# josebeo2016/SCL-Deepfake-audio-detection

Measured on AMD Instinct MI355X. Metric: train-step utterances/sec (64000-sample clips), higher is better.
Workload: dtype bf16

## Files before the change

### scl-deepfake-audio-detection_amd/csrc/gemm.hip

```cpp
#include "gemm_common.h"

using namespace sclg;

namespace {

constexpr int BM = 128, BN = 128;

struct StageK {
    __amdgpu_buffer_rsrc_t rsrc;
    unsigned rowoff[4];
    unsigned lds_off[4];
    int kcur, kend;

    __device__ __forceinline__ void init(const OpK& o, const char* base, int row0, int rowlimit, int kbegin, int kend_, int tid) {
        rsrc = make_rsrc(base);
        const int c = tid & 7;
#pragma unroll
        for (int i = 0; i < 4; ++i) {
            const int row = (tid >> 3) + 32 * i;
            const int r = row0 + row;
            rowoff[i] = r < rowlimit ? row_off(o, (unsigned)r) : OOB;
            lds_off[i] = (unsigned)(row * 128 + ((c ^ ((row >> 1) & 7)) << 4));
        }
        kcur = kbegin + 8 * c; kend = kend_;
// ... 644 lines not shown

bool fill_operand(const SclOperand& o, const char* name, long long rows, long long contig, OpK* k, int esz) {
    const int vec = 16 / esz;
    if (!o.ptr || ((uintptr_t)o.ptr & 15)) { scl_set_error("gemm: %s ptr null or not 16B aligned", name); return false; }
    if (o.rpb < 1 || o.cin < vec) { scl_set_error("gemm: %s rpb/cin invalid", name); return false; }
    if ((o.ld % vec) || (o.rbstride % vec) || (o.cout % vec) || (o.bs1 % vec) || (o.bs2 % vec) || (o.cin != 0x7fffffff && (o.cin % vec))) {
        scl_set_error("gemm: %s strides must be multiples of %d elements", name, vec); return false;
    }
    const long long rq = (rows - 1) / o.rpb, rr = o.rpb == 0x7fffffff ? rows - 1 : (long long)o.rpb - 1;
    const long long cq = o.cin == 0x7fffffff ? 0 : (contig - 1) / o.cin;
    const long long cr = o.cin == 0x7fffffff ? contig - 1 : (long long)o.cin - 1;
    const long long maxoff = rq * o.rbstride + (rr < rows - 1 ? rr : rows - 1) * (long long)o.ld + cq * o.cout + cr + vec;
    if (maxoff < 0 || maxoff * esz >= (1ll << 32) - 32 || rows >= (1ll << 31)) {
        scl_set_error("gemm: %s extent exceeds 32-bit byte offsets (%lld elements)", name, maxoff); return false;
    }
    k->ptr = o.ptr; k->bs1 = o.bs1 * esz; k->bs2 = o.bs2 * esz;
    k->rb_bytes = (unsigned)(o.rbstride * esz); k->ld_bytes = (unsigned)o.ld * (unsigned)esz; k->cout_bytes = (unsigned)(o.cout * esz);
    k->rpb = (unsigned)o.rpb; make_magic((unsigned)o.rpb, &k->rpb_magic, &k->rpb_shift);
    k->cin = (unsigned)o.cin; make_magic((unsigned)o.cin, &k->cin_magic, &k->cin_mshift);
    k->esz_shift = esz == 4 ? 2u : 1u;
    return true;
}
}

namespace {

bool gemm_pick_w8(const GemmK& k, bool at, bool bt, const SclGemmDesc& d, long long zdim, W8Plan* plan) {
    const int w8_env = 1;
    if (d.flags & (SCL_GEMM_NO_W8 | SCL_GEMM_FORCE_P8 | SCL_GEMM_FORCE_BIG | SCL_GEMM_NO_DMA)) return false;
    const bool a_whole = at ? (d.M % 8 == 0) : (d.K % 8 == 0);
    const bool b_whole = bt ? (d.N % 8 == 0) : (d.K % 8 == 0);
    static const int ncu_env = [] { const char* e = getenv("SCL_GEMM_CUS"); const int v = e ? atoi(e) : 256; return v >= 32 && v <= 256 ? v : 256; }();
    if (!a_whole || !b_whole || !scl_gemm_w8_plan(k, at, bt, d, zdim, ncu_env, plan)) return false;
    const long long need = at ? 128 : 160;
    return (d.flags & SCL_GEMM_FORCE_W8) || (w8_env && d.N >= 192 && plan->tiles * zdim >= need);
}

#ifdef SCL_EXPERIMENTS
bool gemm_pick_x2(const GemmK& k, bool at, bool bt, const SclGemmDesc& d, long long zdim, W8Plan* plan) {
    static const int x2_env = [] { const char* e = getenv("SCL_GEMM_X2"); return e ? atoi(e) : 0; }();
    if (d.flags & (SCL_GEMM_NO_X2 | SCL_GEMM_FORCE_W8 | SCL_GEMM_FORCE_P8 | SCL_GEMM_FORCE_BIG | SCL_GEMM_NO_DMA)) return false;
    if (!(d.flags & SCL_GEMM_FORCE_X2) && x2_env == 0) return false;
    const bool a_whole = at ? (d.M % 8 == 0) : (d.K % 8 == 0);
    const bool b_whole = bt ? (d.N % 8 == 0) : (d.K % 8 == 0);
    static const int ncu_env = [] { const char* e = getenv("SCL_GEMM_CUS"); const int v = e ? atoi(e) : 256; return v >= 32 && v <= 256 ? v : 256; }();
    if (!a_whole || !b_whole || !scl_gemm_x2_plan(k, at, bt, d, zdim, ncu_env, plan)) return false;
    if ((d.flags & SCL_GEMM_FORCE_X2) || x2_env == 2) return true;
    return !at && d.N >= 128 && plan->tiles * zdim >= 248;
}

#else
bool gemm_pick_x2(const GemmK&, bool, bool, const SclGemmDesc&, long long, W8Plan*) { return false; }
#endif
}

extern "C" int scl_gemm_uses_wide_tiles(const SclGemmDesc* dp) {
    if (!dp || dp->M <= 0 || dp->N <= 0 || dp->K <= 0 || dp->nb1 < 1 || dp->nb2 < 1 || dp->splitk < 1) return 0;
    GemmK k; W8Plan plan;
    const bool at = dp->flags & SCL_GEMM_A_T, bt = dp->flags & SCL_GEMM_B_T;
    const long long zdim = (long long)dp->nb1 * dp->nb2 * dp->splitk;
    if (gemm_pick_x2(k, at, bt, *dp, zdim, &plan)) return 3;
    return gemm_pick_w8(k, at, bt, *dp, zdim, &plan) ? (plan.variant == 2 ? 4 : 1 + plan.variant) : 0;
}

static int gemm_colsum_rows(const SclGemmDesc& d) {
    if (d.M <= 0 || d.N <= 0 || d.K <= 0 || d.nb1 != 1 || d.nb2 != 1 || d.splitk != 1 || (d.N & 7) || (d.ldc & 7) || (d.flags & SCL_GEMM_AB_F32)) return 0;
    GemmK k; W8Plan plan;
    const bool at = d.flags & SCL_GEMM_A_T, bt = d.flags & SCL_GEMM_B_T;
    const bool a_whole = at ? (d.M % 8 == 0) : (d.K % 8 == 0), b_whole = bt ? (d.N % 8 == 0) : (d.K % 8 == 0);
    SclGemmDesc dq = d;
    if (!dq.colsum_part) dq.colsum_part = reinterpret_cast<float*>(16);
    if (!a_whole || !b_whole || (d.flags & SCL_GEMM_NO_DMA) || gemm_pick_x2(k, at, bt, dq, 1, &plan) || !gemm_pick_w8(k, at, bt, dq, 1, &plan)) return 0;
    return plan.tiles_m * 4;
}
extern "C" int scl_gemm_colsum_rows(const SclGemmDesc* dp) { return dp ? gemm_colsum_rows(*dp) : 0; }

static int gemm_fill_k(const SclGemmDesc& d, GemmK& k) {
    SCL_REQUIRE(d.M > 0 && d.N > 0 && d.K > 0, "gemm: M,N,K must be positive (%d,%d,%d)", d.M, d.N, d.K);
    SCL_REQUIRE(d.nb1 >= 1 && d.nb2 >= 1 && d.splitk >= 1, "gemm: nb1/nb2/splitk must be >= 1");
    const bool at = d.flags & SCL_GEMM_A_T, bt = d.flags & SCL_GEMM_B_T;
    const bool f32ab = d.flags & SCL_GEMM_AB_F32;
    if (!f32ab) {
        if (!fill_operand(d.A, "A", at ? d.K : d.M, at ? d.M : d.K, &k.A, 2)) return SCL_EINVAL;
        if (!fill_operand(d.B, "B", bt ? d.K : d.N, bt ? d.N : d.K, &k.B, 2)) return SCL_EINVAL;
    }
    SCL_REQUIRE(d.C && d.c_rpb >= 1, "gemm: C null or c_rpb < 1");
    const int rmode = (d.flags >> SCL_GEMM_RMODE_SHIFT) & 0xF;
    SCL_REQUIRE(rmode == 0 || d.R, "gemm: RMODE set but R is null");
    SCL_REQUIRE(!(d.flags & SCL_GEMM_HAS_C2) || d.C2, "gemm: HAS_C2 set but C2 is null");
    SCL_REQUIRE(!(d.flags & SCL_GEMM_HAS_BIAS) || d.bias, "gemm: HAS_BIAS set but bias is null");
    SCL_REQUIRE(d.splitk == 1 || ((d.flags & SCL_GEMM_C_F32) && rmode == 0 && !(d.flags & (SCL_GEMM_HAS_BIAS | SCL_GEMM_HAS_C2))
                                  && ((d.flags >> SCL_GEMM_ACT_SHIFT) & 0xF) == 0),
                "gemm: split-K needs a plain f32 slab output");
    const long long zdim = (long long)d.nb1 * d.nb2 * d.splitk;
    SCL_REQUIRE(zdim <= 65535, "gemm: batch*splitk too large (%lld)", zdim);
// ... 99 lines not shown
        return scl_check_launch("scl_gemm_bf16(f32 operands)");
    }
    {
        SclProfScope prof(SCL_KID_GEMM, s, 2.0 * d.M * d.N * (double)d.K * d.nb1 * d.nb2, true);
        const bool a_whole = at ? (d.M % 8 == 0) : (d.K % 8 == 0);
        const bool b_whole = bt ? (d.N % 8 == 0) : (d.K % 8 == 0);
        const bool dma = a_whole && b_whole && !(d.flags & SCL_GEMM_NO_DMA);
#ifdef SCL_EXPERIMENTS
        const long long big_tiles = (long long)((d.M + BIG_BM - 1) / BIG_BM) * ((d.N + BN - 1) / BN) * zdim;
        const bool big = dma && (d.flags & SCL_GEMM_FORCE_BIG) && !(d.flags & SCL_GEMM_NO_BIG) && d.M >= 256 && d.K >= 192 && big_tiles >= 1;
        const long long p8_tiles = (long long)((d.M + P8_BM - 1) / P8_BM) * ((d.N + P8_BN - 1) / P8_BN) * zdim;
        const bool p8 = dma && (d.flags & SCL_GEMM_FORCE_P8) && !(d.flags & SCL_GEMM_NO_P8);
#else
        const bool big = false, p8 = false;
#endif
        W8Plan plan;
#ifdef SCL_EXPERIMENTS
        const bool x2 = dma && gemm_pick_x2(k, at, bt, d, zdim, &plan);
#else
        const bool x2 = false;
#endif
        const bool w8 = !x2 && dma && gemm_pick_w8(k, at, bt, d, zdim, &plan);
        if (((unsigned)d.flags & SCL_GEMM_C_SPLIT3) && !w8) {
            scl_set_error("gemm: C_SPLIT3 is served by the wide-tile kernel only, and this launch (M %d, N %d, K %d) does not qualify for it", d.M, d.N, d.K);
            return SCL_EUNSUPPORTED;
        }
#ifdef SCL_EXPERIMENTS
        const char* deep_env = getenv("SCL_GEMM_DEEP");
        const bool deep = !x2 && !w8 && dma && deep_env && atoi(deep_env) != 0 && (long long)tiles * zdim <= 256 && (d.K + BK - 1) / BK / d.splitk >= 4;
#else
        const bool deep = false;
#endif
        const bool w8p = w8 && scl_gemm_w8_persist_blocks(k, at, bt, plan, zdim) > 0;
        prof.note(d.M, d.N, d.K, d.flags, (int)zdim, x2 ? 3 : (w8p ? 8 : (w8 ? (plan.variant == 2 ? 6 : 1 + plan.variant) : (deep ? 7 : 0))));
        if (x2) {
#ifdef SCL_EXPERIMENTS
            scl_gemm_x2_launch(k, at, bt, plan, zdim, s);
#endif
        } else if (w8) {
            scl_gemm_w8_launch(k, at, bt, plan, zdim, s);
#ifdef SCL_EXPERIMENTS
        } else if (p8) {
            static bool p8_attr_set = false;
            if (!p8_attr_set) {
                hipFuncSetAttribute((const void*)scl_gemm_p8_kernel<false, false>, hipFuncAttributeMaxDynamicSharedMemorySize, P8_LDS);
                hipFuncSetAttribute((const void*)scl_gemm_p8_kernel<false, true>, hipFuncAttributeMaxDynamicSharedMemorySize, P8_LDS);
                hipFuncSetAttribute((const void*)scl_gemm_p8_kernel<true, false>, hipFuncAttributeMaxDynamicSharedMemorySize, P8_LDS);
                hipFuncSetAttribute((const void*)scl_gemm_p8_kernel<true, true>, hipFuncAttributeMaxDynamicSharedMemorySize, P8_LDS);
                p8_attr_set = true;
            }
            dim3 pgrid((unsigned)(p8_tiles / zdim), 1, (unsigned)zdim), pblock(512);
            if (!at && !bt) SCL_LAUNCH((scl_gemm_p8_kernel<false, false>), pgrid, pblock, P8_LDS, s, k);
            else if (!at && bt) SCL_LAUNCH((scl_gemm_p8_kernel<false, true>), pgrid, pblock, P8_LDS, s, k);
            else if (at && !bt) SCL_LAUNCH((scl_gemm_p8_kernel<true, false>), pgrid, pblock, P8_LDS, s, k);
            else SCL_LAUNCH((scl_gemm_p8_kernel<true, true>), pgrid, pblock, P8_LDS, s, k);
        } else if (big) {
            static bool attr_set = false;
            if (!attr_set) {
                hipFuncSetAttribute((const void*)scl_gemm_big_kernel<false, false>, hipFuncAttributeMaxDynamicSharedMemorySize, BIG_LDS);
                hipFuncSetAttribute((const void*)scl_gemm_big_kernel<false, true>, hipFuncAttributeMaxDynamicSharedMemorySize, BIG_LDS);
                hipFuncSetAttribute((const void*)scl_gemm_big_kernel<true, false>, hipFuncAttributeMaxDynamicSharedMemorySize, BIG_LDS);
                hipFuncSetAttribute((const void*)scl_gemm_big_kernel<true, true>, hipFuncAttributeMaxDynamicSharedMemorySize, BIG_LDS);
                attr_set = true;
            }
            dim3 bgrid(((d.M + BIG_BM - 1) / BIG_BM) * ((d.N + BN - 1) / BN), 1, (unsigned)zdim), bblock(512);
            if (!at && !bt) SCL_LAUNCH((scl_gemm_big_kernel<false, false>), bgrid, bblock, BIG_LDS, s, k);
            else if (!at && bt) SCL_LAUNCH((scl_gemm_big_kernel<false, true>), bgrid, bblock, BIG_LDS, s, k);
// ... 138 lines not shown
```

### scl-deepfake-audio-detection_amd/csrc/gemm_w8.hip

```cpp
#include "gemm_common.h"
#include "gemm_w8_epi.h"

using namespace sclg;

__device__ unsigned long long scl_gemm_stamps[4096 * 8];

namespace {

__device__ __forceinline__ void w8_stamp(const GemmK& d, int slot, int lane, int wave) {
    if ((d.flags & SCL_GEMM_STAMPS) && wave == 0 && lane == 0 && blockIdx.x < 4096 && blockIdx.z == 0) {
        scl_gemm_stamps[blockIdx.x * 8 + 2 * slot] = __builtin_amdgcn_s_memrealtime();
        scl_gemm_stamps[blockIdx.x * 8 + 2 * slot + 1] = __builtin_amdgcn_s_memtime();
    }
}

constexpr int W8_BN = 256;
constexpr int W8_OPB = 2 * TILE_BYTES;
constexpr int W8_NA = 3, W8_NB = 2;
constexpr int W8_LDS = (W8_NA + W8_NB) * W8_OPB;

struct W8K {
    __amdgpu_buffer_rsrc_t rsrc;
    unsigned voff[4];
    __device__ __forceinline__ void init(const OpK& o, const char* base, int row0, int rowlimit, int lane, int wave) {
        rsrc = make_rsrc(base);
#pragma unroll
        for (int i = 0; i < 4; ++i) {
            const int row = 8 * (wave * 4 + i) + (lane >> 3);
            const int r = row0 + row;
            const int kc = (lane & 7) ^ ((row >> 1) & 7);
            voff[i] = r < rowlimit ? row_off(o, (unsigned)r) + (unsigned)(kc << 4) : OOB;
        }
    }
    template <int I0>
    __device__ __forceinline__ void issue2(char* img, int wave, unsigned soff, bool live) const {
#pragma unroll
        for (int i = I0; i < I0 + 2; ++i) {
            const unsigned off = live ? voff[i] : OOB;
            __builtin_amdgcn_raw_ptr_buffer_load_lds(rsrc, (lds_void*)(img + (wave * 4 + i) * 1024), 16, off, soff, 0, 0);
        }
    }
    __device__ __forceinline__ void issue1(char* img, int wave, unsigned soff, bool live, int i) const {
        const unsigned off = live ? voff[i] : OOB;
        __builtin_amdgcn_raw_ptr_buffer_load_lds(rsrc, (lds_void*)(img + (wave * 4 + i) * 1024), 16, off, soff, 0, 0);
    }
    __device__ __forceinline__ static unsigned kstep(const OpK& o) { return o.cin == 64 ? o.cout_bytes : 128u; }
    __device__ __forceinline__ void rows(const OpK&, int, int, int) {}
    __device__ __forceinline__ void set_batched(bool) {}
    __device__ __forceinline__ unsigned step(const OpK& o) const { return kstep(o); }
};
struct W8T {
    __amdgpu_buffer_rsrc_t rsrc;
    unsigned voff[4];
    int col0_, collimit_;
    bool batched;
    __device__ __forceinline__ void set_batched(bool b) { batched = b; }
    __device__ __forceinline__ void init(const OpK& o, const char* base, int col0, int collimit, int lane, int wave) {
        rsrc = make_rsrc(base);
        col0_ = col0; collimit_ = collimit;
        const int s16 = lane & 15;
#pragma unroll
        for (int i = 0; i < 4; ++i) {
            const int p = wave * 4 + i;
            const int kr = 4 * (p & 15) + (lane >> 4);
            const int sw = (kr & 3) | (((kr >> 3) & 1) << 2);
            const int col = col0 + (p >> 4) * 128 + 8 * ((((s16 >> 1) ^ sw) << 1) | (s16 & 1));
            voff[i] = col < collimit ? (unsigned)kr * o.ld_bytes + col_off(o, (unsigned)col) : OOB;
        }
    }
    __device__ __forceinline__ void rows(const OpK& o, int krow, int lane, int wave) {
        if (!batched) return;
        const int s16 = lane & 15;
#pragma unroll
        for (int i = 0; i < 4; ++i) {
            const int p = wave * 4 + i;
            const int kr = 4 * (p & 15) + (lane >> 4);
            const int sw = (kr & 3) | (((kr >> 3) & 1) << 2);
            const int col = col0_ + (p >> 4) * 128 + 8 * ((((s16 >> 1) ^ sw) << 1) | (s16 & 1));
            voff[i] = col < collimit_ ? row_off(o, (unsigned)(krow + kr)) + col_off(o, (unsigned)col) : OOB;
        }
    }
    template <int I0>
    __device__ __forceinline__ void issue2(char* img, int wave, unsigned soff, bool live) const {
#pragma unroll
        for (int i = I0; i < I0 + 2; ++i) {
            const unsigned off = live ? voff[i] : OOB;
            __builtin_amdgcn_raw_ptr_buffer_load_lds(rsrc, (lds_void*)(img + (wave * 4 + i) * 1024), 16, off, soff, 0, 0);
        }
    }
    __device__ __forceinline__ void issue1(char* img, int wave, unsigned soff, bool live, int i) const {
        const unsigned off = live ? voff[i] : OOB;
        __builtin_amdgcn_raw_ptr_buffer_load_lds(rsrc, (lds_void*)(img + (wave * 4 + i) * 1024), 16, off, soff, 0, 0);
    }
    __device__ __forceinline__ static unsigned kstep(const OpK& o) { return 64u * o.ld_bytes; }
    __device__ __forceinline__ unsigned step(const OpK& o) const { return batched ? 0u : kstep(o); }
};
template <bool T> struct W8Sel { typedef W8K type; };
template <> struct W8Sel<true> { typedef W8T type; };

template <bool T>
__device__ __forceinline__ bf16x8 w8_frag(const char* img, int gb, int ks, int lane) {
    if (T) return frag_t_raw(img + (gb >> 3) * TILE_BYTES, gb & 7, ks, lane);
    return frag_k(img, gb, ks, lane);
}

#define W8_MFMA_PHASE(MH, NH, FBSEL, NI)                                                                   \
    asm volatile("s_waitcnt lgkmcnt(0)" ::: "memory");                                                     \
    __builtin_amdgcn_sched_barrier(0);                                                                     \
    __builtin_amdgcn_s_barrier();                                                                          \
    __builtin_amdgcn_sched_barrier(0);                                                                     \
    __builtin_amdgcn_s_setprio(1);                                                                         \
    _Pragma("unroll") for (int ks = 0; ks < 2; ++ks)                                                       \
        _Pragma("unroll") for (int i = 0; i < (NI); ++i)                                                   \
            _Pragma("unroll") for (int j = 0; j < 2; ++j)                                                  \
                acc[MH][i][2 * (NH) + j] = __builtin_amdgcn_mfma_f32_16x16x32_bf16(FBSEL[j][ks], fa[i][ks], acc[MH][i][2 * (NH) + j], 0, 0, 0); \
    __builtin_amdgcn_s_setprio(0);                                                                         \
    __builtin_amdgcn_sched_barrier(0);                                                                     \
    __builtin_amdgcn_s_barrier();

template <bool AT, bool BT, int NH>
__device__ __forceinline__ void w8_body(const GemmK& d, char* smem, typename W8Sel<AT>::type& la, typename W8Sel<BT>::type& lb,
                                        int nk, unsigned soffA, unsigned soffB, int ab, int m0, int n0, int mlimit,
                                        int z1, int z2, int ksplit, int lane, int wave, int wc, int krow0) {
    const unsigned stepA = la.step(d.A), stepB = lb.step(d.B);
// ... 144 lines not shown
        if constexpr (R < REND) {
            if constexpr (R == 0 || (R > RBW)) {
                constexpr int j = R == 0 ? 0 : R - RBW;
                if constexpr (BT) FB[j] = frag_t_raw(TB + ((nbk + j) >> 3) * TILE_BYTES, (nbk + j) & 7, ks, lane);
                else if constexpr (RAW) FB[j] = lds_b128_raw<j * 2048>(kb);
                else FB[j] = frag_k(TB, nbk + j, ks, lane);
            } else {
                constexpr int i = R - 1;
                if constexpr (AT) FA[i] = frag_t_raw(TA + ((ab + i) >> 3) * TILE_BYTES, (ab + i) & 7, ks, lane);
                else if constexpr (RAW) FA[i] = lds_b128_raw<i * 2048>(ka);
                else FA[i] = frag_k(TA, ab + i, ks, lane);
            }
            if (RAW) __builtin_amdgcn_sched_barrier(0);
            step<R + 1, REND>(FA, FB, TA, TB, ka, kb, ab, nbk, ks, lane);
        }
    }
    template <int R0, int R1, bool ORDERED>
    static __device__ __forceinline__ void go(bf16x8 (&FA)[RBW], bf16x8 (&FB)[4], const char* TA, const char* TB, int ab, int nbk, int ks, int lane) {
        if constexpr (R0 < R1) {
            unsigned ka = 0, kb = 0;
            if constexpr (RAW && !AT) ka = kaddr(TA, ab, ks, lane);
            if constexpr (RAW && !BT) kb = kaddr(TB, nbk, ks, lane);
            if constexpr (ORDERED && !RAW) {
                step<R0, R0 + 1>(FA, FB, TA, TB, ka, kb, ab, nbk, ks, lane);
                __builtin_amdgcn_sched_barrier(0);
                go<R0 + 1, R1, true>(FA, FB, TA, TB, ab, nbk, ks, lane);
            } else {
                step<R0, R1>(FA, FB, TA, TB, ka, kb, ab, nbk, ks, lane);
            }
        }
    }
};

template <bool AT, bool BT, int RBW>
__device__ __forceinline__ void w8s_body(const GemmK& d, char* smem, const typename W8Sel<AT>::type& la, const typename W8Sel<BT>::type& lb,
                                         int nk, unsigned soffA, unsigned soffB, int ab, int m0, int n0, int mlimit,
                                         int z1, int z2, int ksplit, int lane, int wave, int wc) {
    const unsigned stepA = W8Sel<AT>::type::kstep(d.A), stepB = W8Sel<BT>::type::kstep(d.B);
    f32x4 acc[RBW][4];
#pragma unroll
    for (int i = 0; i < RBW; ++i)
#pragma unroll
        for (int j = 0; j < 4; ++j) acc[i][j] = f32x4{0.f, 0.f, 0.f, 0.f};
    bf16x8 fa0[RBW], fa1[RBW], fb0[4], fb1[4];
    const int nbk = wc * 4;
    char* const bimg = smem + W8_NA * W8_OPB;
    char *a_cur = smem, *a_nxt = smem + W8_OPB, *a_fill = smem + 2 * W8_OPB;
    constexpr int NRD = RBW + 4, OPA = AT ? 2 : 1, OPB = BT ? 2 : 1;
    constexpr int RQ0 = NRD < 4 ? NRD : 4, RQ1 = NRD < 8 ? NRD : 8, RQ2 = NRD;
    typedef W8SRead<AT, BT, RBW> RD;
    auto ops_upto = [](int n) constexpr { return (n > 0 ? OPB : 0) + (n > 1 ? (n - 1 < RBW ? n - 1 : RBW) * OPA : 0) + (n > RBW + 1 ? (n - RBW - 1) * OPB : 0); };
    lds_wait_upto(0);
    __builtin_amdgcn_sched_barrier(0);
    RD::template go<0, NRD, true>(fa0, fb0, a_cur, bimg, ab, nbk, 0, lane);
    for (int kt = 0; kt < nk; ++kt) {
        char* tB = bimg + (kt & 1) * W8_OPB;
        const bool live2 = kt + 2 < nk;
#ifdef W8S_FAKE_A
        const bool live2a = false;
#else
        const bool live2a = live2;
#endif
#ifdef W8S_FAKE_B
        const bool live2b = false;
#else
        const bool live2b = live2;
#endif
        soffA += stepA; soffB += stepB;
#define W8S_Q_FIRST(j, R0, R1)                                                                                               \
        RD::template go<R0, R1, false>(fa1, fb1, a_cur, tB, ab, nbk, 1, lane);                                               \
        __builtin_amdgcn_sched_barrier(0);                                                                                   \
        lds_wait_upto((3 - (j)) * OPB + ops_upto(R1));                                                                       \
        __builtin_amdgcn_sched_barrier(0);                                                                                   \
        _Pragma("unroll") for (int i = 0; i < RBW; ++i)                                                                      \
            acc[i][j] = __builtin_amdgcn_mfma_f32_16x16x32_bf16(fb0[j], fa0[i], acc[i][j], 0, 0, 0);                         \
        __builtin_amdgcn_sched_barrier(0);                                                                                   \
        la.issue1(a_fill, wave, soffA, live2a, j);                                                                           \
        __builtin_amdgcn_sched_barrier(0);
        W8S_Q_FIRST(0, 0, RQ0) W8S_Q_FIRST(1, RQ0, RQ1) W8S_Q_FIRST(2, RQ1, RQ2) W8S_Q_FIRST(3, RQ2, NRD)
#undef W8S_Q_FIRST
        lds_wait_upto(0);
        asm volatile("s_waitcnt vmcnt(4)" ::: "memory");
        __builtin_amdgcn_sched_barrier(0);
        __builtin_amdgcn_s_barrier();
        __builtin_amdgcn_sched_barrier(0);
        const char* tBn = bimg + ((kt & 1) ^ 1) * W8_OPB;
#define W8S_B_ISSUE(j) if ((j) < 2) { lb.issue1(tB, wave, soffB, live2b, 2 * (j)); lb.issue1(tB, wave, soffB, live2b, 2 * (j) + 1); }
#define W8S_Q_SECOND(j, R0, R1)                                                                                              \
        RD::template go<R0, R1, false>(fa0, fb0, a_nxt, tBn, ab, nbk, 0, lane);                                              \
        __builtin_amdgcn_sched_barrier(0);                                                                                   \
        _Pragma("unroll") for (int i = 0; i < RBW; ++i)                                                                      \
            acc[i][j] = __builtin_amdgcn_mfma_f32_16x16x32_bf16(fb1[j], fa1[i], acc[i][j], 0, 0, 0);                         \
        __builtin_amdgcn_sched_barrier(0);                                                                                   \
        W8S_B_ISSUE(j)                                                                                                       \
        __builtin_amdgcn_sched_barrier(0);
        W8S_Q_SECOND(0, 0, RQ0) W8S_Q_SECOND(1, RQ0, RQ1) W8S_Q_SECOND(2, RQ1, RQ2) W8S_Q_SECOND(3, RQ2, NRD)
#undef W8S_Q_SECOND
#undef W8S_B_ISSUE
        char* t = a_cur; a_cur = a_nxt; a_nxt = a_fill; a_fill = t;
    }
    asm volatile("s_waitcnt vmcnt(0)" ::: "memory");
    asm volatile("s_waitcnt lgkmcnt(0)" ::: "memory");
    __builtin_amdgcn_s_barrier();
    w8_stamp(d, 2, lane, wave);
    {
        const long long cbase = z1 * d.c_bs1 + z2 * d.c_bs2 + (long long)ksplit * d.c_split_stride;
        const float* bias = (d.flags & SCL_GEMM_HAS_BIAS) ? d.bias + z2 * d.bias_bs2 : nullptr;
        char* wlds = smem + wave * 16384;
        char* wextra = smem + 8 * 16384 + wave * 4096;
        float* cs0 = d.colsum ? d.colsum + ((long long)(m0 / d.tile_m) * 4 + (wave >> 2) * 2) * d.N : nullptr;
        if constexpr (RBW >= 4) {
            f32x4 (&alo)[4][4] = *reinterpret_cast<f32x4 (*)[4][4]>(&acc[0]);
            w8_epilogue_pass<4, ((RBW < 8 && !AT) ? 0x1E : 0)>(d, alo, 4, wlds, wextra, m0 + ab * 16, n0 + wc * 64, mlimit, cbase, bias, lane, cs0);
        } else {
            f32x4 lo[4][4];
#pragma unroll
            for (int i = 0; i < 4; ++i)
#pragma unroll
                for (int j = 0; j < 4; ++j) lo[i][j] = (i < RBW) ? acc[(i < RBW) ? i : 0][j] : f32x4{0.f, 0.f, 0.f, 0.f};
            w8_epilogue_pass<4, ((RBW < 8 && !AT) ? 0x1E : 0)>(d, lo, RBW, wlds, wextra, m0 + ab * 16, n0 + wc * 64, mlimit, cbase, bias, lane, cs0);
        }
        if (RBW > 4) {
            f32x4 hi[4][4];
#pragma unroll
            for (int i = 0; i < 4; ++i)
#pragma unroll
                for (int j = 0; j < 4; ++j) hi[i][j] = (4 + i < RBW) ? acc[(4 + i < RBW) ? 4 + i : 0][j] : f32x4{0.f, 0.f, 0.f, 0.f};
            w8_epilogue_pass<4, ((RBW < 8 && !AT) ? 0x1E : 0)>(d, hi, RBW - 4, wlds, wextra, m0 + (ab + 4) * 16, n0 + wc * 64, mlimit, cbase, bias, lane, cs0 ? cs0 + d.N : nullptr);
        }
    }
    if (d.flags & SCL_GEMM_STAMPS) {
        asm volatile("s_waitcnt vmcnt(0)" ::: "memory");
// ... 25 lines not shown
    const int kt0 = ksplit * nk_per;
    const int nk = max(0, min(nk_per, nk_total - kt0));
    const char* Ab = reinterpret_cast<const char*>(d.A.ptr) + z1 * d.A.bs1 + z2 * d.A.bs2;
    const char* Bb = reinterpret_cast<const char*>(d.B.ptr) + z1 * d.B.bs1 + z2 * d.B.bs2;

    typename W8Sel<AT>::type la;
    typename W8Sel<BT>::type lb;
    la.init(d.A, Ab, m0, mlimit, lane, wave);
    lb.init(d.B, Bb, n0, d.N, lane, wave);
    la.set_batched(false); lb.set_batched(false);
    const unsigned stepA = W8Sel<AT>::type::kstep(d.A), stepB = W8Sel<BT>::type::kstep(d.B);
    unsigned soffA = (unsigned)kt0 * stepA, soffB = (unsigned)kt0 * stepB;
    la.template issue2<0>(smem, wave, soffA, nk > 0); la.template issue2<2>(smem, wave, soffA, nk > 0);
    lb.template issue2<0>(smem + W8_NA * W8_OPB, wave, soffB, nk > 0); lb.template issue2<2>(smem + W8_NA * W8_OPB, wave, soffB, nk > 0);
    soffA += stepA; soffB += stepB;
    la.template issue2<0>(smem + W8_OPB, wave, soffA, nk > 1); la.template issue2<2>(smem + W8_OPB, wave, soffA, nk > 1);
    lb.template issue2<0>(smem + (W8_NA + 1) * W8_OPB, wave, soffB, nk > 1); lb.template issue2<2>(smem + (W8_NA + 1) * W8_OPB, wave, soffB, nk > 1);
    asm volatile("s_waitcnt vmcnt(8)" ::: "memory");
    w8_stamp(d, 1, lane, wave);
    __builtin_amdgcn_s_barrier();
    if (RB0 == RB1) {
        w8s_body<AT, BT, RB0>(d, smem, la, lb, nk, soffA, soffB, wr * RB0, m0, n0, mlimit, z1, z2, ksplit, lane, wave, wc);
    } else if (wr == 0) {
        w8s_body<AT, BT, RB0>(d, smem, la, lb, nk, soffA, soffB, 0, m0, n0, mlimit, z1, z2, ksplit, lane, wave, wc);
    } else {
        w8s_body<AT, BT, RB1>(d, smem, la, lb, nk, soffA, soffB, RB0, m0, n0, mlimit, z1, z2, ksplit, lane, wave, wc);
    }
}

template <bool AT, bool BT, int RB0, int RB1>
__global__ __launch_bounds__(512, 2) void scl_gemm_w8s_kernel(const GemmK d) {
    extern __shared__ __attribute__((aligned(16))) char smem[];
    w8s_tile<AT, BT, RB0, RB1>(d, smem, blockIdx.x, gridDim.x, blockIdx.z);
}

struct GemmGroupK {
    GemmK k[W8_GROUP_MAX];
    int first[W8_GROUP_MAX + 1];
    int tile0[W8_GROUP_MAX];
    int ntiles[W8_GROUP_MAX];
    int n;
    int xcd_major;
};
typedef const __attribute__((address_space(4))) GemmGroupK* W8GArg;
template <bool AT, bool BT, int RB0, int RB1>
__global__ __launch_bounds__(512, 2) void scl_gemm_w8s_group_kernel(const GemmGroupK g) {
    extern __shared__ __attribute__((aligned(16))) char smem[];
    W8GArg gp = (W8GArg)__builtin_amdgcn_kernarg_segment_ptr();
    const int total = g.first[W8_GROUP_MAX];
    const int x = blockIdx.x & 7, idx = blockIdx.x >> 3, q = total >> 3, r = total & 7;
#ifdef SCL_EXPERIMENTS
    const int pos = (g.xcd_major ? ((x < r ? x * (q + 1) : r * (q + 1) + (x - r) * q) + idx) : (int)blockIdx.x);
#else
    const int pos = (x < r ? x * (q + 1) : r * (q + 1) + (x - r) * q) + idx;
#endif
    int mem = 0;
#pragma unroll
    for (int i = 1; i < W8_GROUP_MAX; ++i) mem += (i < g.n && pos >= g.first[i]) ? 1 : 0;
    mem = __builtin_amdgcn_readfirstlane(mem);
    const int t = __builtin_amdgcn_readfirstlane(pos - gp->first[mem] + gp->tile0[mem]);
#ifdef SCL_EXPERIMENTS
    if (!g.xcd_major) { w8s_tile<AT, BT, RB0, RB1, false>(*(const GemmK*)&gp->k[mem], smem, t, gp->ntiles[mem], 0); return; }
#endif
    w8s_tile<AT, BT, RB0, RB1, true>(*(const GemmK*)&gp->k[mem], smem, t, gp->ntiles[mem], 0);
}

// ... 199 lines not shown
        (void)hipFuncSetAttribute((const void*)scl_gemm_w8s_kernel<true, false, RB0, RB1>, hipFuncAttributeMaxDynamicSharedMemorySize, W8_LDS);
        (void)hipFuncSetAttribute((const void*)scl_gemm_w8s_kernel<true, true, RB0, RB1>, hipFuncAttributeMaxDynamicSharedMemorySize, W8_LDS);
        attr_set = true;
    }
    const dim3 block(512);
    if (mode == 1) {
        if (!at && !bt) SCL_LAUNCH((scl_gemm_w8s_kernel<false, false, RB0, RB1>), grid, block, W8_LDS, s, k);
        else if (!at && bt) SCL_LAUNCH((scl_gemm_w8s_kernel<false, true, RB0, RB1>), grid, block, W8_LDS, s, k);
        else if (at && !bt) SCL_LAUNCH((scl_gemm_w8s_kernel<true, false, RB0, RB1>), grid, block, W8_LDS, s, k);
        else SCL_LAUNCH((scl_gemm_w8s_kernel<true, true, RB0, RB1>), grid, block, W8_LDS, s, k);
        return;
    }
    if (!at && !bt) SCL_LAUNCH((scl_gemm_w8_kernel<false, false, RB0, RB1>), grid, block, W8_LDS, s, k);
    else if (!at && bt) SCL_LAUNCH((scl_gemm_w8_kernel<false, true, RB0, RB1>), grid, block, W8_LDS, s, k);
    else if (at && !bt) SCL_LAUNCH((scl_gemm_w8_kernel<true, false, RB0, RB1>), grid, block, W8_LDS, s, k);
    else SCL_LAUNCH((scl_gemm_w8_kernel<true, true, RB0, RB1>), grid, block, W8_LDS, s, k);
}

void w8_launch_43(const GemmK& k, bool bt, dim3 grid, hipStream_t s) {
    static bool attr_set = false;
    if (!attr_set) {
        (void)hipFuncSetAttribute((const void*)scl_gemm_w8s_kernel<false, false, 4, 3>, hipFuncAttributeMaxDynamicSharedMemorySize, W8_LDS);
        (void)hipFuncSetAttribute((const void*)scl_gemm_w8s_kernel<false, true, 4, 3>, hipFuncAttributeMaxDynamicSharedMemorySize, W8_LDS);
        attr_set = true;
    }
    if (!bt) SCL_LAUNCH((scl_gemm_w8s_kernel<false, false, 4, 3>), grid, dim3(512), W8_LDS, s, k);
    else SCL_LAUNCH((scl_gemm_w8s_kernel<false, true, 4, 3>), grid, dim3(512), W8_LDS, s, k);
}

}

namespace sclg {

bool scl_gemm_w8_plan(const GemmK& k, bool at, bool bt, const SclGemmDesc& d, long long zdim, int ncu, W8Plan* plan) {
    auto flat_rows = [](const SclOperand& o, long long rows) { return (long long)o.rpb >= rows; };
    const bool tt = at && bt;
    const bool a_ok = at ? (flat_rows(d.A, d.K) || (tt && d.A.rpb >= 1)) : (d.A.cin == 0x7fffffff || d.A.cin == 64 || d.A.cin >= d.K);
    const bool b_ok = bt ? (flat_rows(d.B, d.K) || (tt && d.B.rpb >= 1)) : (d.B.cin == 0x7fffffff || d.B.cin == 64 || d.B.cin >= d.K);
    if (!a_ok || !b_ok || (d.K % BK) != 0) return false;
    const long long tiles_n = (d.N + W8_BN - 1) / W8_BN;
    long long best = -1;
    const char* e43 = getenv("SCL_W8_TILE112");
    const char* epp = getenv("SCL_W8_MODE");
    const bool v43_env = !e43 || atoi(e43) != 0, pingpong_env = epp && *epp && atoi(epp) == 0;
    const bool v43_ok = v43_env && !pingpong_env && !at && zdim == 1 && !d.colsum_part && !(d.flags & SCL_GEMM_STAMPS);
    for (int v = 0; v < (v43_ok ? 3 : 2); ++v) {
        const int bm = v == 0 ? 208 : (v == 1 ? 256 : 112);
        const long long ntm = (d.M + bm - 1) / bm;
        const long long rounds = (ntm * tiles_n * zdim + ncu - 1) / ncu;
        const long long cost = rounds * (bm + W8_BN);
        if (best < 0 || cost < best) {
            best = cost;
            plan->variant = v; plan->tiles_m = (int)ntm; plan->tile_m = (int)((d.M + ntm - 1) / ntm);
            plan->tiles = ntm * tiles_n; plan->cost = cost; plan->ncu = ncu;
        }
    }
    return true;
}

bool scl_gemm_w8_group_member_ok(const GemmK& k, bool at, bool bt, const SclGemmDesc& d) {
    if (!at || !bt || d.nb1 != 1 || d.nb2 != 1 || d.splitk != 1 || (d.K % BK) != 0 || d.K / BK < 3) return false;
    if ((long long)d.A.rpb < (long long)d.K || (long long)d.B.rpb < (long long)d.K) return false;
    if ((d.M % 8) || (d.N % 8) || !k.vec_ok) return false;
    const int plain = SCL_GEMM_A_T | SCL_GEMM_B_T | SCL_GEMM_C_F32;
    return (d.flags & ~(SCL_GEMM_NO_DMA | SCL_GEMM_NO_W8)) == plain && !d.colsum_part;
}

// ... 36 lines not shown
int scl_gemm_read_stamps(unsigned long long* out, int nblocks) {
    return hipMemcpyFromSymbol(out, HIP_SYMBOL(scl_gemm_stamps), sizeof(unsigned long long) * 8 * (size_t)nblocks) == hipSuccess ? 0 : -1;
}

int scl_gemm_w8_persist_blocks(const GemmK& k, bool at, bool bt, const W8Plan& plan, long long zdim) {
    const char* pe = getenv("SCL_W8_PERSIST");
    const int pv = (pe && *pe) ? atoi(pe) : 1;
    const char* me = getenv("SCL_W8_MODE");
    static const bool epi_generic = [] { const char* e = getenv("SCL_W8_EPI_GENERIC"); return e && atoi(e) != 0; }();
    if (pv <= 0 || (me && *me && atoi(me) != 1) || epi_generic) return 0;
    if (plan.variant > 1 || at || zdim != 1 || k.splitk != 1 || k.K / BK < 3 || (k.flags & SCL_GEMM_STAMPS)) return 0;
    const int ek = w8p_epi_kind(k.flags);
    if (!ek || !w8p_built(bt, ek, plan.variant) || ((unsigned)k.flags & SCL_GEMM_C_SPLIT3) || !k.vec_ok || (k.ldc & 7) || (k.c_rbstride & 7)) return 0;
    if (pv >= 8) return pv > 256 ? 256 : (pv & ~7);
    const long long ncu = plan.ncu >= 8 ? plan.ncu : 256;
    const long long rounds = (plan.tiles + ncu - 1) / ncu;
    long long G = (((plan.tiles + rounds - 1) / rounds) + 7) & ~7ll;
    if (G > (ncu & ~7ll)) G = ncu & ~7ll;
    return (G >= 8 && plan.tiles >= 2 * G) ? (int)G : 0;
}

int scl_gemm_w8_launch(GemmK& k, bool at, bool bt, const W8Plan& plan, long long zdim, hipStream_t s) {
    k.tile_m = plan.tile_m;
    k.debug = 0;
    {
        const long long nb1 = zdim / ((long long)k.nb2 * k.splitk);
        const long long rows = k.M - 1, rpb = (long long)k.c_rpb;
        const long long maxoff = (nb1 - 1) * k.c_bs1 + ((long long)k.nb2 - 1) * k.c_bs2 + (rows / rpb) * k.c_rbstride + (rows % rpb) * k.ldc + k.N;
        if (maxoff * ((k.flags & SCL_GEMM_R_F32) ? 4 : 2) >= 0xFFFFFF00ll) k.debug |= 2;
    }
    const dim3 grid((unsigned)plan.tiles, 1, (unsigned)zdim);
    const char* me = getenv("SCL_W8_MODE");
    int mode = (me && *me) ? atoi(me) : 1;
    if (at && bt) {
        if ((long long)k.A.rpb < (long long)k.K) { k.debug |= 4; mode = 0; }
        if ((long long)k.B.rpb < (long long)k.K) { k.debug |= 8; mode = 0; }
    }
    {
        static const bool epi_generic = [] { const char* e = getenv("SCL_W8_EPI_GENERIC"); return e && atoi(e) != 0; }();
        if (epi_generic) k.debug |= 16;
    }
    dim3 g = grid;
#ifdef SCL_EXPERIMENTS
    {
        const char* sg = getenv("SCL_W8_STAGGER");
        const int stg = sg ? atoi(sg) : 0;
        if (stg > 0 && plan.tiles > 256 && zdim == 1) k.debug |= (stg & 0xFF) << 8;
    }
#endif
    if (mode == 1) {
        const int G = scl_gemm_w8_persist_blocks(k, at, bt, plan, zdim);
        if (G > 0) {
            ++w8p_launches;
            w8p_launch(k, bt, w8p_epi_kind(k.flags), plan.variant, dim3((unsigned)G, 1, 1), s);
            return 0;
        }
    }
    if (plan.variant == 2) w8_launch_43(k, bt, g, s);
    else if (plan.variant == 0) w8_launch_rb<7, 6>(k, at, bt, g, s, mode);
    else w8_launch_rb<8, 8>(k, at, bt, g, s, mode);
    return 0;
}

}
```

Before: 1666.

## Add segmented-K wide-tile GEMM kernel for transposed batched-row operands

```diff
diff --git a/scl-deepfake-audio-detection_amd/csrc/gemm.hip b/scl-deepfake-audio-detection_amd/csrc/gemm.hip
--- a/scl-deepfake-audio-detection_amd/csrc/gemm.hip
+++ b/scl-deepfake-audio-detection_amd/csrc/gemm.hip
@@ -700,6 +700,7 @@
     const bool b_whole = bt ? (d.N % 8 == 0) : (d.K % 8 == 0);
     static const int ncu_env = [] { const char* e = getenv("SCL_GEMM_CUS"); const int v = e ? atoi(e) : 256; return v >= 32 && v <= 256 ? v : 256; }();
     if (!a_whole || !b_whole || !scl_gemm_w8_plan(k, at, bt, d, zdim, ncu_env, plan)) return false;
+    if (plan->variant == 3) return true;
     const long long need = at ? 128 : 160;
     return (d.flags & SCL_GEMM_FORCE_W8) || (w8_env && d.N >= 192 && plan->tiles * zdim >= need);
 }
@@ -728,7 +729,7 @@
     const bool at = dp->flags & SCL_GEMM_A_T, bt = dp->flags & SCL_GEMM_B_T;
     const long long zdim = (long long)dp->nb1 * dp->nb2 * dp->splitk;
     if (gemm_pick_x2(k, at, bt, *dp, zdim, &plan)) return 3;
-    return gemm_pick_w8(k, at, bt, *dp, zdim, &plan) ? (plan.variant == 2 ? 4 : 1 + plan.variant) : 0;
+    return gemm_pick_w8(k, at, bt, *dp, zdim, &plan) ? (plan.variant == 3 ? 5 : (plan.variant == 2 ? 4 : 1 + plan.variant)) : 0;
 }
 
 static int gemm_colsum_rows(const SclGemmDesc& d) {
@@ -894,7 +895,7 @@
         const bool deep = false;
 #endif
         const bool w8p = w8 && scl_gemm_w8_persist_blocks(k, at, bt, plan, zdim) > 0;
-        prof.note(d.M, d.N, d.K, d.flags, (int)zdim, x2 ? 3 : (w8p ? 8 : (w8 ? (plan.variant == 2 ? 6 : 1 + plan.variant) : (deep ? 7 : 0))));
+        prof.note(d.M, d.N, d.K, d.flags, (int)zdim, x2 ? 3 : (w8p ? 8 : (w8 ? (plan.variant == 3 ? 9 : (plan.variant == 2 ? 6 : 1 + plan.variant)) : (deep ? 7 : 0))));
         if (x2) {
 #ifdef SCL_EXPERIMENTS
             scl_gemm_x2_launch(k, at, bt, plan, zdim, s);
diff --git a/scl-deepfake-audio-detection_amd/csrc/gemm_w8.hip b/scl-deepfake-audio-detection_amd/csrc/gemm_w8.hip
--- a/scl-deepfake-audio-detection_amd/csrc/gemm_w8.hip
+++ b/scl-deepfake-audio-detection_amd/csrc/gemm_w8.hip
@@ -53,11 +53,13 @@
     __amdgpu_buffer_rsrc_t rsrc;
     unsigned voff[4];
     int col0_, collimit_;
+    int kq_;
     bool batched;
     __device__ __forceinline__ void set_batched(bool b) { batched = b; }
     __device__ __forceinline__ void init(const OpK& o, const char* base, int col0, int collimit, int lane, int wave) {
         rsrc = make_rsrc(base);
         col0_ = col0; collimit_ = collimit;
+        kq_ = lane >> 4;
         const int s16 = lane & 15;
 #pragma unroll
         for (int i = 0; i < 4; ++i) {
@@ -90,6 +92,11 @@
     }
     __device__ __forceinline__ void issue1(char* img, int wave, unsigned soff, bool live, int i) const {
         const unsigned off = live ? voff[i] : OOB;
+        __builtin_amdgcn_raw_ptr_buffer_load_lds(rsrc, (lds_void*)(img + (wave * 4 + i) * 1024), 16, off, soff, 0, 0);
+    }
+    __device__ __forceinline__ void issue1r(char* img, int wave, unsigned soff, int rows, int i) const {
+        const int thr = rows - 16 * (wave & 3) - 4 * i;
+        const unsigned off = kq_ < thr ? voff[i] : OOB;
         __builtin_amdgcn_raw_ptr_buffer_load_lds(rsrc, (lds_void*)(img + (wave * 4 + i) * 1024), 16, off, soff, 0, 0);
     }
     __device__ __forceinline__ static unsigned kstep(const OpK& o) { return 64u * o.ld_bytes; }
@@ -300,10 +307,21 @@
     }
 };
 
-template <bool AT, bool BT, int RBW>
+struct W8Seg {
+    int st, nst, rem;
+    unsigned baseA, baseB;
+    unsigned rbA, rbB;
+    __device__ __forceinline__ void next() {
+        if (++st == nst) { st = 0; baseA += rbA; baseB += rbB; }
+    }
+    __device__ __forceinline__ int rows() const { return st + 1 == nst ? rem : BK; }
+};
+
+template <bool AT, bool BT, int RBW, bool SEG = false>
 __device__ __forceinline__ void w8s_body(const GemmK& d, char* smem, const typename W8Sel<AT>::type& la, const typename W8Sel<BT>::type& lb,
                                          int nk, unsigned soffA, unsigned soffB, int ab, int m0, int n0, int mlimit,
-                                         int z1, int z2, int ksplit, int lane, int wave, int wc) {
+                                         int z1, int z2, int ksplit, int lane, int wave, int wc, W8Seg cur = W8Seg()) {
+    static_assert(!SEG || (AT && BT), "w8s_body: the segmented K loop reads transposed operands");
     const unsigned stepA = W8Sel<AT>::type::kstep(d.A), stepB = W8Sel<BT>::type::kstep(d.B);
     f32x4 acc[RBW][4];
 #pragma unroll
@@ -334,7 +352,14 @@
 #else
         const bool live2b = live2;
 #endif
-        soffA += stepA; soffB += stepB;
+        int rows2 = 0;
+        if constexpr (SEG) {
+            cur.next();
+            soffA = cur.baseA + (unsigned)cur.st * stepA; soffB = cur.baseB + (unsigned)cur.st * stepB;
+            rows2 = live2 ? cur.rows() : 0;
+        } else {
+            soffA += stepA; soffB += stepB;
+        }
 #define W8S_Q_FIRST(j, R0, R1)                                                                                               \
         RD::template go<R0, R1, false>(fa1, fb1, a_cur, tB, ab, nbk, 1, lane);                                               \
         __builtin_amdgcn_sched_barrier(0);                                                                                   \
@@ -343,7 +368,8 @@
         _Pragma("unroll") for (int i = 0; i < RBW; ++i)                                                                      \
             acc[i][j] = __builtin_amdgcn_mfma_f32_16x16x32_bf16(fb0[j], fa0[i], acc[i][j], 0, 0, 0);                         \
         __builtin_amdgcn_sched_barrier(0);                                                                                   \
-        la.issue1(a_fill, wave, soffA, live2a, j);                                                                           \
+        if constexpr (SEG) la.issue1r(a_fill, wave, soffA, rows2, j);                                                        \
+        else la.issue1(a_fill, wave, soffA, live2a, j);                                                                      \
         __builtin_amdgcn_sched_barrier(0);
         W8S_Q_FIRST(0, 0, RQ0) W8S_Q_FIRST(1, RQ0, RQ1) W8S_Q_FIRST(2, RQ1, RQ2) W8S_Q_FIRST(3, RQ2, NRD)
 #undef W8S_Q_FIRST
@@ -353,7 +379,9 @@
         __builtin_amdgcn_s_barrier();
         __builtin_amdgcn_sched_barrier(0);
         const char* tBn = bimg + ((kt & 1) ^ 1) * W8_OPB;
-#define W8S_B_ISSUE(j) if ((j) < 2) { lb.issue1(tB, wave, soffB, live2b, 2 * (j)); lb.issue1(tB, wave, soffB, live2b, 2 * (j) + 1); }
+#define W8S_B_ISSUE(j) if ((j) < 2) {                                                                                        \
+            if constexpr (SEG) { lb.issue1r(tB, wave, soffB, rows2, 2 * (j)); lb.issue1r(tB, wave, soffB, rows2, 2 * (j) + 1); }     \
+            else { lb.issue1(tB, wave, soffB, live2b, 2 * (j)); lb.issue1(tB, wave, soffB, live2b, 2 * (j) + 1); } }
 #define W8S_Q_SECOND(j, R0, R1)                                                                                              \
         RD::template go<R0, R1, false>(fa0, fb0, a_nxt, tBn, ab, nbk, 0, lane);                                              \
         __builtin_amdgcn_sched_barrier(0);                                                                                   \
@@ -366,6 +394,10 @@
 #undef W8S_Q_SECOND
 #undef W8S_B_ISSUE
         char* t = a_cur; a_cur = a_nxt; a_nxt = a_fill; a_fill = t;
+    }
+    if constexpr (SEG) {
+        lds_wait_upto(0);
+        __builtin_amdgcn_sched_barrier(0);
     }
     asm volatile("s_waitcnt vmcnt(0)" ::: "memory");
     asm volatile("s_waitcnt lgkmcnt(0)" ::: "memory");
@@ -457,6 +489,55 @@
 __global__ __launch_bounds__(512, 2) void scl_gemm_w8s_kernel(const GemmK d) {
     extern __shared__ __attribute__((aligned(16))) char smem[];
     w8s_tile<AT, BT, RB0, RB1>(d, smem, blockIdx.x, gridDim.x, blockIdx.z);
+}
+
+template <int RB0, int RB1>
+__global__ __launch_bounds__(512, 2) void scl_gemm_segk_w8_kernel(const GemmK d) {
+    static_assert(RB0 == RB1, "w8s seg: equal wave rows");
+    extern __shared__ __attribute__((aligned(16))) char smem[];
+    const int tid = threadIdx.x, lane = tid & 63;
+    const int wave = __builtin_amdgcn_readfirstlane(tid >> 6);
+    const int wr = wave >> 2, wc = wave & 3;
+    const int tiles_m = d.M / d.tile_m, ntile = tiles_m * (d.N / W8_BN);
+    const int total = gridDim.x;
+    const int x = blockIdx.x & 7, idx = blockIdx.x >> 3, q = total >> 3, r = total & 7;
+    const int pos = (x < r ? x * (q + 1) : r * (q + 1) + (x - r) * q) + idx;
+    const int ksplit = __builtin_amdgcn_readfirstlane(pos / ntile);
+    const int t = pos - ksplit * ntile;
+    const int tn = __builtin_amdgcn_readfirstlane(t / tiles_m), tm = t - tn * tiles_m;
+    const int m0 = tm * d.tile_m, n0 = tn * W8_BN, mlimit = m0 + d.tile_m;
+    W8Seg cur;
+    const int T = (int)d.A.rpb;
+    cur.nst = (T + BK - 1) / BK;
+    cur.rem = T - (cur.nst - 1) * BK;
+    const int nk_total = __builtin_amdgcn_readfirstlane(d.K / T) * cur.nst;
+    const int nk_per = __builtin_amdgcn_readfirstlane((nk_total + d.splitk - 1) / d.splitk);
+    const int kt0 = ksplit * nk_per;
+    const int nk = max(0, min(nk_per, nk_total - kt0));
+    const int u0 = __builtin_amdgcn_readfirstlane(kt0 / cur.nst);
+    cur.st = kt0 - u0 * cur.nst;
+    cur.rbA = d.A.rb_bytes; cur.rbB = d.B.rb_bytes;
+    cur.baseA = (unsigned)u0 * cur.rbA; cur.baseB = (unsigned)u0 * cur.rbB;
+
+    W8T la, lb;
+    la.init(d.A, reinterpret_cast<const char*>(d.A.ptr), m0, mlimit, lane, wave);
+    lb.init(d.B, reinterpret_cast<const char*>(d.B.ptr), n0, d.N, lane, wave);
+    la.set_batched(false); lb.set_batched(false);
+    const unsigned stepA = W8T::kstep(d.A), stepB = W8T::kstep(d.B);
+    char* const bimg = smem + W8_NA * W8_OPB;
+#pragma unroll
+    for (int s = 0; s < 2; ++s) {
+        const int rows = nk > s ? cur.rows() : 0;
+        const unsigned soffA = cur.baseA + (unsigned)cur.st * stepA, soffB = cur.baseB + (unsigned)cur.st * stepB;
+#pragma unroll
+        for (int i = 0; i < 4; ++i) la.issue1r(smem + s * W8_OPB, wave, soffA, rows, i);
+#pragma unroll
+        for (int i = 0; i < 4; ++i) lb.issue1r(bimg + s * W8_OPB, wave, soffB, rows, i);
+        if (s == 0) cur.next();
+    }
+    asm volatile("s_waitcnt vmcnt(8)" ::: "memory");
+    __builtin_amdgcn_s_barrier();
+    w8s_body<true, true, RB0, true>(d, smem, la, lb, nk, 0u, 0u, wr * RB0, m0, n0, mlimit, 0, 0, ksplit, lane, wave, wc, cur);
 }
 
 struct GemmGroupK {
@@ -722,7 +803,27 @@
 
 namespace sclg {
 
+static bool w8_seg_ok(bool at, bool bt, const SclGemmDesc& d) {
+    const char* se = getenv("SCL_W8_SEGK");
+    const char* me = getenv("SCL_W8_MODE");
+    const int sv = (se && *se) ? atoi(se) : 1;
+    if (sv <= 0 || (me && *me && atoi(me) != 1)) return false;
+    if (!at || !bt || d.nb1 != 1 || d.nb2 != 1 || d.colsum_part) return false;
+    if (d.A.rpb != d.B.rpb || (long long)d.A.rpb > (long long)d.K || (d.K % d.A.rpb) != 0) return false;
+    if ((d.M % 256) || (d.N % W8_BN)) return false;
+    if (sv < 2 && ((long long)(d.M / 256) * (d.N / W8_BN) < 12 || (d.flags & SCL_GEMM_FORCE_W8))) return false;
+    if (d.A.cin != 0x7fffffff || d.B.cin != 0x7fffffff) return false;
+    const int plain = SCL_GEMM_A_T | SCL_GEMM_B_T | SCL_GEMM_C_F32;
+    const bool strides4 = !(d.ldc & 3) && !(d.c_rbstride & 3) && !(d.c_split_stride & 3) && ((uintptr_t)d.C & 15) == 0;
+    return (d.flags & ~(SCL_GEMM_NO_X2 | SCL_GEMM_NO_BIG | SCL_GEMM_NO_P8 | SCL_GEMM_FORCE_W8)) == plain && strides4;
+}
+
 bool scl_gemm_w8_plan(const GemmK& k, bool at, bool bt, const SclGemmDesc& d, long long zdim, int ncu, W8Plan* plan) {
+    if (w8_seg_ok(at, bt, d)) {
+        plan->variant = 3; plan->tiles_m = d.M / 256; plan->tile_m = 256;
+        plan->tiles = (long long)plan->tiles_m * (d.N / W8_BN); plan->cost = 0; plan->ncu = ncu;
+        return true;
+    }
     auto flat_rows = [](const SclOperand& o, long long rows) { return (long long)o.rpb >= rows; };
     const bool tt = at && bt;
     const bool a_ok = at ? (flat_rows(d.A, d.K) || (tt && d.A.rpb >= 1)) : (d.A.cin == 0x7fffffff || d.A.cin == 64 || d.A.cin >= d.K);
@@ -825,7 +926,7 @@
     const dim3 grid((unsigned)plan.tiles, 1, (unsigned)zdim);
     const char* me = getenv("SCL_W8_MODE");
     int mode = (me && *me) ? atoi(me) : 1;
-    if (at && bt) {
+    if (at && bt && plan.variant != 3) {
         if ((long long)k.A.rpb < (long long)k.K) { k.debug |= 4; mode = 0; }
         if ((long long)k.B.rpb < (long long)k.K) { k.debug |= 8; mode = 0; }
     }
@@ -849,7 +950,14 @@
             return 0;
         }
     }
-    if (plan.variant == 2) w8_launch_43(k, bt, g, s);
+    if (plan.variant == 3) {
+        static bool attr_set = false;
+        if (!attr_set) {
+            (void)hipFuncSetAttribute((const void*)scl_gemm_segk_w8_kernel<8, 8>, hipFuncAttributeMaxDynamicSharedMemorySize, W8_LDS);
+            attr_set = true;
+        }
+        SCL_LAUNCH((scl_gemm_segk_w8_kernel<8, 8>), dim3((unsigned)(plan.tiles * zdim)), dim3(512), W8_LDS, s, k);
+    } else if (plan.variant == 2) w8_launch_43(k, bt, g, s);
     else if (plan.variant == 0) w8_launch_rb<7, 6>(k, at, bt, g, s, mode);
     else w8_launch_rb<8, 8>(k, at, bt, g, s, mode);
     return 0;
```

After: 1676 (median of 6 runs). Within noise of the previous version (+0.6%).
